# mmetcalf14/qml-cutensornet

Measured on AMD Instinct MI355X. Metric: Gram kernel entries/sec @ 60 qubits x 6 layers, higher is better.
Workload: dtype f64 (complex128)

## Files before the change

qml-cutensornet_amd/csrc/qk_fused.h:

```cpp
#pragma once
#include "qk_device.h"
#include "qk_plan.h"

#define QKF_PRIO_LO() __builtin_amdgcn_s_setprio(0)
#define QKF_PRIO_HI() __builtin_amdgcn_s_setprio(2)
typedef double v2d __attribute__((ext_vector_type(2)));
typedef __attribute__((address_space(3))) v2d lds_v2d;
static constexpr int QKF_XSTEP = 4 * TILE;
static constexpr int QKF_XBLOCK = TILE * TILE;


#ifndef QKF_LDS3M
#define QKF_LDS3M 0
#endif
#ifndef QKF_P2_PROBE
#define QKF_P2_PROBE 0
#endif
#ifndef QKF_ABL
#define QKF_ABL 0
#endif
#define QKF_STEP_BARRIER()                            \
  do {                                                \
    if (QKF_ABL & 4) asm volatile("s_waitcnt lgkmcnt(0)" ::: "memory"); \
    else qk_lds_barrier();                            \
// ... 79 lines not shown
    bo += bs, xq.advance();
#pragma unroll
    for (int i = 0; i < 4; ++i) {
      if (i == 0) {
        const v4d z = {0, 0, 0, 0};
        p1 = __builtin_amdgcn_mfma_f64_16x16x4f64(fx[0].x, fr[0].x, z, 0, 0, 0);
        p2 = __builtin_amdgcn_mfma_f64_16x16x4f64(fx[0].y, fr[0].y, z, 0, 0, 0);
        p3 = __builtin_amdgcn_mfma_f64_16x16x4f64(QKF_SUM(fx[0].x, fx[0].y), QKF_SUM(fr[0].x, fr[0].y), z, 0, 0, 0);
      } else {
        qkf_kstep<false>(p1, p2, p3, fx[i].x, fx[i].y, fr[i].x, fr[i].y);
      }
      if (!(QKF_ABL & 2)) fr[i] = qkf_ldgb(cb[i], bo);
      if (!(QKF_ABL & 8)) fx[i] = xq.kstep(i);
      __builtin_amdgcn_sched_barrier(0);
    }
  }
#pragma unroll 1
  for (int pass = 0; pass < 2; ++pass) {
    const int end = ng - 2 + pass;
#pragma unroll 1
    for (; gq < end; ++gq) {
      bo += bs, xq.advance();
#pragma unroll
      for (int i = 0; i < 4; ++i) {
        qkf_kstep<false>(p1, p2, p3, fx[i].x, fx[i].y, fr[i].x, fr[i].y);
        if (!(QKF_ABL & 2)) fr[i] = qkf_ldgb(cb[i], bo);
        if (!(QKF_ABL & 8)) fx[i] = xq.kstep(i);
        __builtin_amdgcn_sched_barrier(0);
      }
    }
#pragma unroll
    for (int i = 0; i < 4; ++i) cb[i] = qkf_kbase(cur.base, cur.step, i, last);
  }
#pragma unroll
  for (int i = 0; i < 4; ++i) {
    if (i < last) qkf_kstep<false>(p1, p2, p3, fx[i].x, fx[i].y, fr[i].x, fr[i].y);
    if (!(QKF_ABL & 2)) fr[i] = qkf_ldg(qkf_kbase(nxt.base, nxt.step, i, nxt.lim), nxt.off);
    __builtin_amdgcn_sched_barrier(0);
  }
  QKF_PRIO_HI();
  t.re = p1 - p2;
  t.im = p3 - p1 - p2;
}

typedef __attribute__((address_space(3))) int lds_int;
struct QkfTurn {
  lds_int* at;
  int idx;
  lds_int* broken;
  unsigned long long* gerr;
};
__device__ __forceinline__ void qkf_turn_add(__attribute__((address_space(3))) double* const d, const long rs, const v4d& re, const v4d& im, const QkfTurn& t, const int tn) {
  lds_int* const turn = t.at + tn;
  if (t.idx > 0) {
    int spins = 0;
#ifdef QKF_FIRST_STORE
    while (__builtin_amdgcn_readfirstlane(__hip_atomic_load(turn, __ATOMIC_RELAXED, __HIP_MEMORY_SCOPE_WORKGROUP)) == 0) {
#else
    while (__builtin_amdgcn_readfirstlane(__hip_atomic_load(turn, __ATOMIC_RELAXED, __HIP_MEMORY_SCOPE_WORKGROUP)) != t.idx) {
#endif
      __builtin_amdgcn_s_sleep(1);
      if (++spins > (1 << 20) || __builtin_amdgcn_readfirstlane(__hip_atomic_load(t.broken, __ATOMIC_RELAXED, __HIP_MEMORY_SCOPE_WORKGROUP)) != 0) {
        __hip_atomic_store(t.broken, 1, __ATOMIC_RELAXED, __HIP_MEMORY_SCOPE_WORKGROUP);
        if (t.gerr) *t.gerr = 1ull;
        break;
      }
    }
#pragma unroll
    for (int r = 0; r < 4; ++r) {
      __hip_atomic_fetch_add(d + r * rs, re[r], __ATOMIC_RELAXED, __HIP_MEMORY_SCOPE_WORKGROUP);
      __hip_atomic_fetch_add(d + r * rs + 1, im[r], __ATOMIC_RELAXED, __HIP_MEMORY_SCOPE_WORKGROUP);
    }
  } else {
#pragma unroll
    for (int r = 0; r < 4; ++r) *(lds_v2d*)(d + r * rs) = (v2d){re[r], im[r]};
  }
#ifdef QKF_FIRST_STORE
  if (t.idx > 0) return;
#endif
  asm volatile("s_waitcnt lgkmcnt(0)" ::: "memory");
  __hip_atomic_store(turn, t.idx + 1, __ATOMIC_RELAXED, __HIP_MEMORY_SCOPE_WORKGROUP);
}

template <bool FULL, bool DET = false>
__device__ __forceinline__ void qkf_p2_item(const QkfTile& t, v2d (&fr)[4], const bool primed, QkfStream cur, const int ps, const int nn, const int kmax, lds_v2d* xo, const int q,
                                            const int j, const QkfStream nxt, const QkfTurn turn = QkfTurn{nullptr, 0, nullptr, nullptr}) {
  if (!primed) qkf_load4(fr, cur);
  __attribute__((address_space(3))) double* d = (__attribute__((address_space(3))) double*)(xo + q * TILE + j);
  if constexpr (!DET) {
    const v4d z = {0, 0, 0, 0};
    const v4d s = t.re + t.im;
#pragma unroll 1
    for (int tn = 0; tn < nn; ++tn) {
      v4d p1 = z, re, im;
      double sp[4], sm[4];
      const bool fin = tn + 1 == nn;
      const v2d* const rb = fin ? nxt.base : cur.base;
      const int rs = fin ? nxt.step : cur.step, rl = fin ? nxt.lim : FULL ? 4 : kmax;
      cur.off = fin ? nxt.off : cur.off + TILE;
      QKF_PRIO_LO();
#pragma unroll
      for (int i = 0; i < 4; ++i) {
        if (FULL || i == 0 || i < kmax) {
          p1 = __builtin_amdgcn_mfma_f64_16x16x4f64(s[i], fr[i].x, i == 0 ? z : p1, 0, 0, 0);
          sp[i] = QKF_DIF(-fr[i].x, fr[i].y), sm[i] = QKF_DIF(fr[i].y, fr[i].x);
        }
        if (!(QKF_ABL & 2)) fr[i] = qkf_ldg_a(qkf_kbase(rb, rs, i, rl), cur.off);
        __builtin_amdgcn_sched_barrier(0);
      }
#pragma unroll
      for (int i = 0; i < 4; ++i) {
        if (FULL || i == 0 || i < kmax) {
          re = __builtin_amdgcn_mfma_f64_16x16x4f64(t.im[i], sm[i], i == 0 ? p1 : re, 0, 0, 0);
          im = __builtin_amdgcn_mfma_f64_16x16x4f64(t.re[i], sp[i], i == 0 ? p1 : im, 0, 0, 0);
        }
        __builtin_amdgcn_sched_barrier(0);
      }
      QKF_PRIO_HI();
#pragma unroll
      for (int r = 0; r < 4; ++r) {
        __hip_atomic_fetch_add(d + r * 2 * QKF_XSTEP, re[r], __ATOMIC_RELAXED, __HIP_MEMORY_SCOPE_WORKGROUP);
        __hip_atomic_fetch_add(d + r * 2 * QKF_XSTEP + 1, im[r], __ATOMIC_RELAXED, __HIP_MEMORY_SCOPE_WORKGROUP);
      }
      d += 2 * ps;
    }
    return;
  }
#pragma unroll 1
  for (int tn = 0; tn < nn; ++tn) {
    v4d p1 = {0, 0, 0, 0}, p2 = {0, 0, 0, 0}, p3 = {0, 0, 0, 0};
    const bool fin = tn + 1 == nn;
    const v2d* const rb = fin ? nxt.base : cur.base;
    const int rs = fin ? nxt.step : cur.step, rl = fin ? nxt.lim : FULL ? 4 : kmax;
    cur.off = fin ? nxt.off : cur.off + TILE;
    QKF_PRIO_LO();
#pragma unroll
    for (int i = 0; i < 4; ++i) {
      if (FULL || i < kmax) qkf_kstep<true>(p1, p2, p3, t.re[i], t.im[i], fr[i].x, fr[i].y);
      if (!(QKF_ABL & 2)) fr[i] = qkf_ldg_a(qkf_kbase(rb, rs, i, rl), cur.off);
      __builtin_amdgcn_sched_barrier(0);
    }
    QKF_PRIO_HI();
    const v4d re = p1 + p2, im = p3 - p1 + p2;
    qkf_turn_add(d, (long)2 * QKF_XSTEP, re, im, turn, tn);
    d += 2 * ps;
  }
}

template <bool HAS1>
__device__ __forceinline__ void qkf_p2_switch(const QkfTile& t0, const QkfTile& t1, v2d (&fr)[4], const bool primed, QkfStream cur, const int lim, const int nn, const int kmax,
                                              __attribute__((address_space(3))) double* d, const int d1off, const QkfStream nxt) {
  if (!primed) qkf_load4(fr, cur);
  const v4d dm0 = t0.im - t0.re, ng0 = -t0.re - t0.im, dm1 = HAS1 ? t1.im - t1.re : dm0, ng1 = HAS1 ? -t1.re - t1.im : ng0;
#pragma unroll 1
  for (int tn = 0; tn < nn; ++tn) {
    v4d p1 = {0, 0, 0, 0}, p2 = {0, 0, 0, 0}, p3 = {0, 0, 0, 0}, r1 = {0, 0, 0, 0}, r2 = {0, 0, 0, 0}, r3 = {0, 0, 0, 0};
    const bool fin = tn + 1 == nn;
    const v2d* const rb = fin ? nxt.base : cur.base;
    const int rs = fin ? nxt.step : cur.step, rl = fin ? nxt.lim : lim;
    cur.off = fin ? nxt.off : cur.off + TILE;
    QKF_PRIO_LO();
#pragma unroll
    for (int i = 0; i < 4; ++i) {
      if (i < kmax) {
        const double sa = QKF_SUM(fr[i].x, fr[i].y);
        p1 = __builtin_amdgcn_mfma_f64_16x16x4f64(sa, t0.re[i], p1, 0, 0, 0);
        p2 = __builtin_amdgcn_mfma_f64_16x16x4f64(fr[i].y, dm0[i], p2, 0, 0, 0);
        p3 = __builtin_amdgcn_mfma_f64_16x16x4f64(fr[i].x, ng0[i], p3, 0, 0, 0);
        if (HAS1) {
          r1 = __builtin_amdgcn_mfma_f64_16x16x4f64(sa, t1.re[i], r1, 0, 0, 0);
          r2 = __builtin_amdgcn_mfma_f64_16x16x4f64(fr[i].y, dm1[i], r2, 0, 0, 0);
          r3 = __builtin_amdgcn_mfma_f64_16x16x4f64(fr[i].x, ng1[i], r3, 0, 0, 0);
        }
      }
      fr[i] = qkf_ldg_a(qkf_kbase(rb, rs, i, rl), cur.off);
      __builtin_amdgcn_sched_barrier(0);
    }
    QKF_PRIO_HI();
    {
      const v4d re = p1 + p2, im = p1 + p3;
#pragma unroll
      for (int r = 0; r < 4; ++r) {
        __hip_atomic_fetch_add(d + r * 2 * QKF_XSTEP, re[r], __ATOMIC_RELAXED, __HIP_MEMORY_SCOPE_WORKGROUP);
        __hip_atomic_fetch_add(d + r * 2 * QKF_XSTEP + 1, im[r], __ATOMIC_RELAXED, __HIP_MEMORY_SCOPE_WORKGROUP);
      }
    }
    if (HAS1) {
      const v4d re = r1 + r2, im = r1 + r3;
#pragma unroll
      for (int r = 0; r < 4; ++r) {
        __hip_atomic_fetch_add(d + d1off + r * 2 * QKF_XSTEP, re[r], __ATOMIC_RELAXED, __HIP_MEMORY_SCOPE_WORKGROUP);
        __hip_atomic_fetch_add(d + d1off + r * 2 * QKF_XSTEP + 1, im[r], __ATOMIC_RELAXED, __HIP_MEMORY_SCOPE_WORKGROUP);
      }
    }
    d += 2 * QKF_XBLOCK;
  }
}

template <int S>
__device__ __forceinline__ void qkf_rotate(QkfTile (&T)[S], const int L) {
  if constexpr (S >= 2) {
    if (L == 2) {
      const QkfTile t = T[S - 2];
      T[S - 2] = T[S - 1], T[S - 1] = t;
    }
  }
  if constexpr (S >= 3) {
    if (L == 3) {
      const QkfTile t = T[S - 3];
      T[S - 3] = T[S - 2], T[S - 2] = T[S - 1], T[S - 1] = t;
    }
  }
  if constexpr (S >= 4) {
    if (L >= 4) {
      const QkfTile t0 = T[0];
#pragma unroll
      for (int e = 0; e + 1 < S; ++e) T[e] = T[e + 1];
      T[S - 1] = t0;
    }
  }
}

#ifdef QKF_EDGE_PAIRS_V
#define QKF_EDGE_PAIRS(WPS) (QKF_EDGE_PAIRS_V != 0)
#else
#define QKF_EDGE_PAIRS(WPS) false
#endif
#ifdef QKF_EDGE_SETS_V
#define QKF_EDGE_SETS(WPS) (QKF_EDGE_SETS_V)
#else
#define QKF_EDGE_SETS(WPS) ((WPS) <= 3 ? 2 : 1)
#endif
__device__ __forceinline__ v2d qkf_lde(const v2d* __restrict__ base, const unsigned boff, const int col = 0) {
  return reinterpret_cast<const v2d*>(reinterpret_cast<const char*>(base) + (size_t)boff)[col];
}
template <bool HAS1, bool MORE>
__device__ __forceinline__ void qkf_edge_group(v4d (&acc)[6], v2d (&fy)[4], v2d (&fz)[4], v2d (&fx)[4], const v2d* const* const by, const v2d* const* const bx, const unsigned boy,
                                               const unsigned box) {
#pragma unroll
  for (int i = 0; i < 4; ++i) {
    const double sb = QKF_DIF(fx[i].x, fx[i].y);
    acc[0] = __builtin_amdgcn_mfma_f64_16x16x4f64(fy[i].x, fx[i].x, acc[0], 0, 0, 0);
    acc[1] = __builtin_amdgcn_mfma_f64_16x16x4f64(fy[i].y, fx[i].y, acc[1], 0, 0, 0);
    acc[2] = __builtin_amdgcn_mfma_f64_16x16x4f64(QKF_SUM(fy[i].x, fy[i].y), sb, acc[2], 0, 0, 0);
    if (HAS1) {
      acc[3] = __builtin_amdgcn_mfma_f64_16x16x4f64(fz[i].x, fx[i].x, acc[3], 0, 0, 0);
      acc[4] = __builtin_amdgcn_mfma_f64_16x16x4f64(fz[i].y, fx[i].y, acc[4], 0, 0, 0);
      acc[5] = __builtin_amdgcn_mfma_f64_16x16x4f64(QKF_SUM(fz[i].x, fz[i].y), sb, acc[5], 0, 0, 0);
    }
    if (MORE) {
      fy[i] = qkf_lde(by[i], boy);
      if (HAS1) fz[i] = qkf_lde(by[i], boy, TILE);
      fx[i] = qkf_lde(bx[i], box);
    }
    __builtin_amdgcn_sched_barrier(0);
  }
}
template <bool HAS1, int SETS>
__device__ __forceinline__ void qkf_edge_unit(QkfTile& t0, QkfTile& t1, const v2d* __restrict__ Ay, const unsigned oy, const int ldy, const v2d* __restrict__ Ax, const unsigned ox, const int ldx,
                                              const int ng) {
  static_assert(SETS == 1 || SETS == 2, "one or two groups of k-steps in flight");
  v4d acc[6];
#pragma unroll
  for (int e = 0; e < 6; ++e) acc[e] = (v4d){0, 0, 0, 0};
  v2d fy[SETS][4], fz[SETS][4], fx[SETS][4];
  const v2d *by[4 * SETS], *bx[4 * SETS];
#pragma unroll
  for (int i = 0; i < 4 * SETS; ++i) by[i] = Ay + 4 * i * ldy, bx[i] = Ax + 4 * i * ldx;
  unsigned boy = oy * 16u, box = ox * 16u;
  const unsigned sy = (unsigned)(SETS * TILE * ldy) * 16u, sx = (unsigned)(SETS * TILE * ldx) * 16u;
  const bool two = SETS == 2 && ng > 1;
#pragma unroll
  for (int s = 0; s < SETS; ++s) {
    if (s == 0 || two) {
#pragma unroll
      for (int i = 0; i < 4; ++i) {
        fy[s][i] = qkf_lde(by[4 * s + i], boy);
        if (HAS1) fz[s][i] = qkf_lde(by[4 * s + i], boy, TILE);
        fx[s][i] = qkf_lde(bx[4 * s + i], box);
// ... 252 lines not shown
    }
    QKF_STAMP(0);
    QkfTile T[S];
    v2d fr[4];
    bool primed = false;
    QkfSite sn = site(ek);
    for (int k = ek; k < k_hi;) {
      const QkfSite sc = sn;
      k = sc.next;
      if (k < k_hi) sn = site(k);
      const int a = sc.a, a2 = sc.a2, b = sc.b, mt = sc.mt, nt = sc.nt, W = sc.W;
      const bool small = sc.small;
      v2d* const Gc = G0 + (long long)cur * g.x_plane;
      v2d* const Gn = G0 + (long long)(cur ^ 1) * g.x_plane;
      if (small && xg) {
        for (int e = tid; e < a * b; e += NT) XL[e] = Gc[e];
        __syncthreads();
        xg = false, xb = 0;
      } else if (!small && !xg) {
        for (int e = tid; e < a * b; e += NT) Gc[e] = XL[xb + e];
        __syncthreads();
        xg = true;
      }
      const int n_out = sc.b2 * a2;
      const bool pingpong = small && a * b + n_out <= XCAP;
      const int ob = !small ? 0 : pingpong ? (xb == 0 ? XCAP - n_out : 0) : 0;
      if (pingpong && !DET)
        for (int e = tid; e < n_out; e += NT) XL[ob + e] = (v2d){0.0, 0.0};
      QKF_STAMP(1);
      for (int s0 = 0; s0 < nt; s0 += W) {
        const int w = min(W, nt - s0), items = sc.pd * mt * w;
        lds_int* const tcur = turn0 + tsel * g.turn_ints;
        if constexpr (DET) {
          for (int e = tid; e < g.turn_ints; e += NT) turn0[(tsel ^ 1) * g.turn_ints + e] = 0;
        } else if (!small) {
          for (int e = tid; e < w * TILE * a2; e += NT) XL[e] = (v2d){0.0, 0.0};
          QKF_STEP_BARRIER();
        }
        QKF_STAMP(6);
        for (int r0 = 0; r0 < items; r0 += NW * S) {
          const int L = min(S, (items - r0 + NW - 1) / NW);
          const bool multi = L > 1;
          const int it0 = r0 + wave;
          auto phase1 = [&](auto xbase) __attribute__((always_inline)) {
#pragma unroll 1
            for (int s = 0; s < L; ++s) {
              if (multi) qkf_rotate<S>(T, L);
              const int it = it0 + NW * s;
              if (it < items) {
                const int ta = item_of(sc, w, it).ta;
                const bool more = s + 1 < L && it + NW < items;
                const QkfStream nxt = more ? b_stream(sc, s0, w, it + NW) : a_stream(sc, w, it0);
                qkf_p1_tile(T[S - 1], fr, primed, b_stream(sc, s0, w, it), xbase, (unsigned)(ta * (b * TILE) + q * TILE + j), sc.nks, nxt);
                primed = true;
              }
            }
          };
          if (xg) phase1((const v2d*)Gc);
          else phase1((const lds_v2d*)(XL + xb));
          QKF_STAMP(2);
          if (small && r0 == 0 && !(DET && pingpong)) {
            QKF_STEP_BARRIER();
            if (!pingpong && !DET) {
              for (int e = tid; e < n_out; e += NT) XL[e] = (v2d){0.0, 0.0};
              QKF_STEP_BARRIER();
            }
          }
          QKF_STAMP(3);
          const bool last_round = s0 + W >= nt && r0 + NW * S >= items;
#pragma unroll 1
          for (int s = 0; s < S; ++s) {
            const int it = it0 + NW * s;
            if (it >= items) break;
            if (multi) qkf_rotate<S>(T, L);
            const QkUnit un = item_of(sc, w, it);
            const int ta = un.ta, tbl = un.tc;
            const int kmax = min(4, (sc.at - ta * TILE + 3) >> 2);
            const bool more = s + 1 < S && it + NW < items;
            const int wn = min(sn.W, sn.nt);
            const bool chain = !more && last_round && k < k_hi && wave < sn.pd * sn.mt * wn;
            const QkfStream nxt = more ? a_stream(sc, w, it + NW) : chain ? b_stream(sn, 0, wn, wave) : a_stream(sc, w, it);
            const int tix = sc.pd * ta + un.p;
            const QkfTurn turn{tcur + tbl * sc.nn, tix, tbroken, g.err};
            if (!DET && sc.sw)
              qkf_p2_switch<false>(T[S - 1], T[S - 1], fr, primed, a_stream(sc, w, it), kmax, sc.nn, kmax, (__attribute__((address_space(3))) double*)(XL + ob + tbl * (a2 * TILE) + q * TILE + j), 0, nxt);
            else if (kmax == 4) qkf_p2_item<true, DET>(T[S - 1], fr, primed, a_stream(sc, w, it), w * QKF_XBLOCK, sc.nn, 4, XL + ob + tbl * QKF_XBLOCK, q, j, nxt, turn);
            else qkf_p2_item<false, DET>(T[S - 1], fr, primed, a_stream(sc, w, it), w * QKF_XBLOCK, sc.nn, kmax, XL + ob + tbl * QKF_XBLOCK, q, j, nxt, turn);
            primed = more || chain;
          }
          QKF_STAMP(4);
        }
        QKF_STEP_BARRIER();
        tsel ^= 1;
        QKF_STAMP(5);
        if (!small && nt > W) {
          for (int tn = 0; tn < sc.nn; ++tn)
            for (int e = tid; e < w * QKF_XBLOCK; e += NT) Gn[(long long)tn * (sc.b2 * TILE) + s0 * QKF_XBLOCK + e] = XL[tn * w * QKF_XBLOCK + e];
          __syncthreads();
          QKF_STAMP(1);
        }
      }
      if (!small) {
        if (nt > W) cur ^= 1;
        else xg = false, xb = 0;
      } else {
        xb = ob;
      }
    }
    const int fl_end = DET ? 0 : rfl(rec[3 * (k_hi - 1) + 1].w);
    const bool sw_end = (fl_end & QK_REC_SWITCH) != 0, o_end = ((fl_end & QK_REC_ORIENT) != 0) != sw_end;
    if (edges) {
      const v4i r0 = rec[3 * (k_hi - 1)];
      const int a_l = rfl(r0.y), b_l = rfl(r0.w), a_e = sw_end ? b_l : a_l, b_e = sw_end ? a_l : b_l;
      qkf_edge_suffix<NW, QKF_EDGE_PAIRS(WPS), QKF_EDGE_SETS(WPS)>(g, o_end ? yj : xi, o_end ? xi : yj, a_e, b_e, (const lds_v2d*)(XL + xb), (const v2d*)(G0 + (long long)cur * g.x_plane), xg, zacc, wave,
                                                                   q, j, o_end);
      __syncthreads();
    }
    if (tid == 0) {
      v2d zz = {0.0, 0.0};
      if (edges)
        for (int w_ = 0; w_ < NW; ++w_) zz.x += zacc[2 * w_], zz.y += zacc[2 * w_ + 1];
      else zz = xg ? G0[(long long)cur * g.x_plane] : (v2d)XL[xb];
      if (o_end) zz.y = -zz.y;
      g.values[p] = zz.x * zz.x + zz.y * zz.y;
      if (g.z) {
        g.z[2 * p] = zz.x;
        g.z[2 * p + 1] = zz.y;
      }
    }
    __syncthreads();
  }
  if (tid == 0) qk_tail_exit(g);
  QKF_PROF_FLUSH();
}

template <bool HAS1, typename XPtr>
__device__ __forceinline__ void qkf_p1_dual(QkfTile& t0, QkfTile& t1, v2d (&fr)[4], v2d (&fs)[4], const bool primed, QkfStream cur, XPtr xp, unsigned xoff, const int nks,
                                            const QkfStream nxt) {
  v4d p1 = {0, 0, 0, 0}, p2 = {0, 0, 0, 0}, p3 = {0, 0, 0, 0}, r1 = {0, 0, 0, 0}, r2 = {0, 0, 0, 0}, r3 = {0, 0, 0, 0};
  v2d fx[4];
  if (!primed) qkf_load4(fr, cur);
  if (HAS1) {
#pragma unroll
    for (int i = 0; i < 4; ++i) fs[i] = qkf_ldg(cur.base + i * cur.step, cur.off + TILE);
  }
#pragma unroll
  for (int i = 0; i < 4; ++i) fx[i] = qkf_ldx(xp + i * QKF_XSTEP, xoff);
  const int ng = (nks + 3) >> 2, last = nks - 4 * (ng - 1);
  QKF_PRIO_LO();
  int gq = 0;
  if (ng >= 2) {
    gq = 1;
    cur.off += 4 * cur.step, xoff += 4 * QKF_XSTEP;
#pragma unroll
    for (int i = 0; i < 4; ++i) {
      if (i == 0) {
        const v4d z = {0, 0, 0, 0};
        const double sa = QKF_SUM(fx[0].x, fx[0].y);
        p1 = __builtin_amdgcn_mfma_f64_16x16x4f64(fx[0].x, fr[0].x, z, 0, 0, 0);
        p2 = __builtin_amdgcn_mfma_f64_16x16x4f64(fx[0].y, fr[0].y, z, 0, 0, 0);
        p3 = __builtin_amdgcn_mfma_f64_16x16x4f64(sa, QKF_SUM(fr[0].x, fr[0].y), z, 0, 0, 0);
        if (HAS1) {
          r1 = __builtin_amdgcn_mfma_f64_16x16x4f64(fx[0].x, fs[0].x, z, 0, 0, 0);
          r2 = __builtin_amdgcn_mfma_f64_16x16x4f64(fx[0].y, fs[0].y, z, 0, 0, 0);
          r3 = __builtin_amdgcn_mfma_f64_16x16x4f64(sa, QKF_SUM(fs[0].x, fs[0].y), z, 0, 0, 0);
        }
      } else {
        qkf_kstep<false>(p1, p2, p3, fx[i].x, fx[i].y, fr[i].x, fr[i].y);
        if (HAS1) qkf_kstep<false>(r1, r2, r3, fx[i].x, fx[i].y, fs[i].x, fs[i].y);
      }
      if (!(QKF_ABL & 2)) fr[i] = qkf_ldg_b(cur.base + i * cur.step, cur.off);
      if (HAS1 && !(QKF_ABL & 2)) fs[i] = qkf_ldg_b(cur.base + i * cur.step, cur.off + TILE);
      if (!(QKF_ABL & 8)) fx[i] = qkf_ldx(xp + i * QKF_XSTEP, xoff);
      __builtin_amdgcn_sched_barrier(0);
    }
  }
#pragma unroll 1
  for (; gq + 1 < ng; ++gq) {
    cur.off += 4 * cur.step, xoff += 4 * QKF_XSTEP;
#pragma unroll
    for (int i = 0; i < 4; ++i) {
      qkf_kstep<false>(p1, p2, p3, fx[i].x, fx[i].y, fr[i].x, fr[i].y);
      if (HAS1) qkf_kstep<false>(r1, r2, r3, fx[i].x, fx[i].y, fs[i].x, fs[i].y);
      if (!(QKF_ABL & 2)) fr[i] = qkf_ldg_b(cur.base + i * cur.step, cur.off);
      if (HAS1 && !(QKF_ABL & 2)) fs[i] = qkf_ldg_b(cur.base + i * cur.step, cur.off + TILE);
      if (!(QKF_ABL & 8)) fx[i] = qkf_ldx(xp + i * QKF_XSTEP, xoff);
      __builtin_amdgcn_sched_barrier(0);
    }
  }
#pragma unroll
  for (int i = 0; i < 4; ++i) {
    if (i < last) {
      qkf_kstep<false>(p1, p2, p3, fx[i].x, fx[i].y, fr[i].x, fr[i].y);
      if (HAS1) qkf_kstep<false>(r1, r2, r3, fx[i].x, fx[i].y, fs[i].x, fs[i].y);
    }
    if (!(QKF_ABL & 2)) fr[i] = qkf_ldg(nxt.base + i * nxt.step, nxt.off);
    __builtin_amdgcn_sched_barrier(0);
  }
  QKF_PRIO_HI();
  t0.re = p1 - p2, t0.im = p3 - p1 - p2;
  if (HAS1) t1.re = r1 - r2, t1.im = r3 - r1 - r2;
}

typedef __attribute__((address_space(3))) double lds_double;
template <bool FULL, bool HAS1>
__device__ __forceinline__ void qkf_p2_block(const QkfTile& t0, const QkfTile& t1, const v4d& s0, const v4d& s1, v2d (&fr)[4], const int kmax, const v2d* const b0, const v2d* const b1,
                                             const v2d* const b2, const v2d* const b3, const unsigned off, lds_double* const d, lds_double* const d1, const long rs) {
  const v4d z = {0, 0, 0, 0};
  v4d p1 = z, r1 = z, re, im, re1, im1;
  double sp[4], sm[4];
  QKF_PRIO_LO();
#pragma unroll
  for (int i = 0; i < 4; ++i) {
    if (FULL || i == 0 || i < kmax) {
      p1 = __builtin_amdgcn_mfma_f64_16x16x4f64(s0[i], fr[i].x, i == 0 ? z : p1, 0, 0, 0);
      if (HAS1) r1 = __builtin_amdgcn_mfma_f64_16x16x4f64(s1[i], fr[i].x, i == 0 ? z : r1, 0, 0, 0);
      sp[i] = QKF_DIF(-fr[i].x, fr[i].y), sm[i] = QKF_DIF(fr[i].y, fr[i].x);
    }
    if (!(QKF_ABL & 2)) fr[i] = qkf_ldg_a(i == 0 ? b0 : i == 1 ? b1 : i == 2 ? b2 : b3, off);
    __builtin_amdgcn_sched_barrier(0);
  }
#pragma unroll
  for (int i = 0; i < 4; ++i) {
    if (FULL || i == 0 || i < kmax) {
      re = __builtin_amdgcn_mfma_f64_16x16x4f64(t0.im[i], sm[i], i == 0 ? p1 : re, 0, 0, 0);
      im = __builtin_amdgcn_mfma_f64_16x16x4f64(t0.re[i], sp[i], i == 0 ? p1 : im, 0, 0, 0);
      if (HAS1) {
        re1 = __builtin_amdgcn_mfma_f64_16x16x4f64(t1.im[i], sm[i], i == 0 ? r1 : re1, 0, 0, 0);
        im1 = __builtin_amdgcn_mfma_f64_16x16x4f64(t1.re[i], sp[i], i == 0 ? r1 : im1, 0, 0, 0);
      }
    }
    __builtin_amdgcn_sched_barrier(0);
  }
  QKF_PRIO_HI();
#pragma unroll
  for (int r = 0; r < 4; ++r) {
    __hip_atomic_fetch_add(d + r * rs, re[r], __ATOMIC_RELAXED, __HIP_MEMORY_SCOPE_WORKGROUP);
    __hip_atomic_fetch_add(d + r * rs + 1, im[r], __ATOMIC_RELAXED, __HIP_MEMORY_SCOPE_WORKGROUP);
  }
  if (HAS1) {
#pragma unroll
    for (int r = 0; r < 4; ++r) {
      __hip_atomic_fetch_add(d1 + r * rs, re1[r], __ATOMIC_RELAXED, __HIP_MEMORY_SCOPE_WORKGROUP);
      __hip_atomic_fetch_add(d1 + r * rs + 1, im1[r], __ATOMIC_RELAXED, __HIP_MEMORY_SCOPE_WORKGROUP);
    }
  }
}
template <bool FULL, bool HAS1, bool DET>
__device__ __forceinline__ void qkf_p2_dual_turn(const QkfTile& t0, const QkfTile& t1, v2d (&fr)[4], v2d (&fs)[4], QkfStream cur, const int ps, const int nn, const int kmax, lds_v2d* xo, const int q,
                                            const int j, const QkfStream nxt, const bool nxt_p1, const unsigned n1, const QkfTurn turn = QkfTurn{nullptr, 0, nullptr, nullptr}) {
  __attribute__((address_space(3))) double* d = (__attribute__((address_space(3))) double*)(xo + q * TILE + j);
#pragma unroll 1
  for (int tn = 0; tn < nn; ++tn) {
    v4d p1 = {0, 0, 0, 0}, p2 = {0, 0, 0, 0}, p3 = {0, 0, 0, 0}, r1 = {0, 0, 0, 0}, r2 = {0, 0, 0, 0}, r3 = {0, 0, 0, 0};
    const bool fin = tn + 1 == nn;
    const v2d* const rb = fin ? nxt.base : cur.base;
    const int rs = fin ? nxt.step : cur.step;
    cur.off = fin ? nxt.off : cur.off + TILE;
    QKF_PRIO_LO();
#pragma unroll
    for (int i = 0; i < 4; ++i) {
      if (FULL || i < kmax) {
        qkf_kstep<true>(p1, p2, p3, t0.re[i], t0.im[i], fr[i].x, fr[i].y);
        if (HAS1) qkf_kstep<true>(r1, r2, r3, t1.re[i], t1.im[i], fr[i].x, fr[i].y);
      }
      fr[i] = qkf_ldg_a(rb + i * rs, cur.off);
      __builtin_amdgcn_sched_barrier(0);
    }
    QKF_PRIO_HI();
    {
      const v4d re = p1 + p2, im = p3 - p1 + p2;
      if constexpr (DET) qkf_turn_add(d, (long)2 * QKF_XSTEP, re, im, turn, tn);
      else {
#pragma unroll
        for (int r = 0; r < 4; ++r) {
          __hip_atomic_fetch_add(d + r * 2 * QKF_XSTEP, re[r], __ATOMIC_RELAXED, __HIP_MEMORY_SCOPE_WORKGROUP);
          __hip_atomic_fetch_add(d + r * 2 * QKF_XSTEP + 1, im[r], __ATOMIC_RELAXED, __HIP_MEMORY_SCOPE_WORKGROUP);
        }
      }
    }
    if (HAS1) {
      const v4d re = r1 + r2, im = r3 - r1 + r2;
      __attribute__((address_space(3))) double* const d1 = d + 2 * QKF_XBLOCK;
      if constexpr (DET) qkf_turn_add(d1, (long)2 * QKF_XSTEP, re, im, QkfTurn{turn.at + nn, turn.idx, turn.broken, turn.gerr}, tn);
      else {
#pragma unroll
        for (int r = 0; r < 4; ++r) {
          __hip_atomic_fetch_add(d1 + r * 2 * QKF_XSTEP, re[r], __ATOMIC_RELAXED, __HIP_MEMORY_SCOPE_WORKGROUP);
          __hip_atomic_fetch_add(d1 + r * 2 * QKF_XSTEP + 1, im[r], __ATOMIC_RELAXED, __HIP_MEMORY_SCOPE_WORKGROUP);
        }
      }
    }
    d += 2 * ps;
  }
}

template <bool FULL, bool HAS1, bool DET = false>
__device__ __forceinline__ void qkf_p2_dual(const QkfTile& t0, const QkfTile& t1, v2d (&fr)[4], v2d (&fs)[4], QkfStream cur, const int ps, const int nn, const int kmax, lds_v2d* xo, const int q,
                                            const int j, const QkfStream nxt, const bool nxt_p1, const unsigned n1, const QkfTurn turn = QkfTurn{nullptr, 0, nullptr, nullptr}) {
  if constexpr (DET) {
    qkf_p2_dual_turn<FULL, HAS1, DET>(t0, t1, fr, fs, cur, ps, nn, kmax, xo, q, j, nxt, nxt_p1, n1, turn);
    return;
  }
  lds_double* d = (lds_double*)(xo + q * TILE + j);
  lds_double* d1 = d + 2 * QKF_XBLOCK;
  constexpr long rs = 2 * QKF_XSTEP;
  const v4d s0 = t0.re + t0.im, s1 = HAS1 ? t1.re + t1.im : s0;
  const v2d *const c0 = cur.base, *const c1 = cur.base + cur.step, *const c2 = cur.base + 2 * cur.step, *const c3 = cur.base + 3 * cur.step;
  unsigned off = cur.off;
#pragma unroll 1
  for (int tn = 0; tn + 1 < nn; ++tn) {
    off += TILE;
    qkf_p2_block<FULL, HAS1>(t0, t1, s0, s1, fr, kmax, c0, c1, c2, c3, off, d, d1, rs);
    d += 2 * ps, d1 += 2 * ps;
  }
  qkf_p2_block<FULL, HAS1>(t0, t1, s0, s1, fr, kmax, nxt.base, nxt.base + nxt.step, nxt.base + 2 * nxt.step, nxt.base + 3 * nxt.step, nxt.off, d, d1, rs);
}

template <int NW, int XCAP, int WPS, bool DET = false>
__global__ __launch_bounds__(64 * NW, WPS) void qk_sweep_fused_dual_kernel(const SweepArgs g) {
  constexpr int NT = 64 * NW;
  extern __shared__ __attribute__((aligned(16))) double lds_raw[];
  lds_v2d* const XL = (lds_v2d*)lds_raw;
  long long* const slot = reinterpret_cast<long long*>(lds_raw + 2 * XCAP);
  const v2d* const xdata = reinterpret_cast<const v2d*>(g.xdata);
  const v2d* const ydata = reinterpret_cast<const v2d*>(g.ydata);
  v2d* const G0 = reinterpret_cast<v2d*>(g.scratch) + (long long)blockIdx.x * 2 * g.x_plane;
  const int tid = threadIdx.x, lane = tid & 63;
  const int wave = __builtin_amdgcn_readfirstlane(tid >> 6);
  const int j = lane & 15, q = lane >> 4;
  const int ns = g.n_sites;
  __attribute__((address_space(3))) double* const zacc = (__attribute__((address_space(3))) double*)(slot + 2);
  lds_v4i* const rec = (lds_v4i*)(slot + 2 + 32);
  long long* const m_off = reinterpret_cast<long long*>(slot + 2 + 32) + 6 * (long long)ns;
  lds_int* const tbroken = (lds_int*)(m_off + 2 * (long long)ns);
  lds_int* const turn0 = tbroken + 2;
  auto rfl = [&](const int v) __attribute__((always_inline)) { return __builtin_amdgcn_readfirstlane(v); };
  auto ldl = [&](const long long* p_) __attribute__((always_inline)) {
    const long long v = *p_;
    const unsigned lo = __builtin_amdgcn_readfirstlane((unsigned)v);
    const unsigned hi = __builtin_amdgcn_readfirstlane((unsigned)((unsigned long long)v >> 32));
    return (long long)(((unsigned long long)hi << 32) | lo);
  };
  auto site = [&](const int k) __attribute__((always_inline)) {
    const v4i r0 = rec[3 * k], r1 = rec[3 * k + 1], r2 = rec[3 * k + 2];
    QkfSite s;
    s.a = rfl(r0.x), s.a2 = rfl(r0.y), s.b = rfl(r0.z), s.b2 = rfl(r0.w);
    s.at = rfl(r1.x), s.nks = rfl(r1.y), s.W = rfl(r1.z), s.small = (rfl(r1.w) & QK_REC_SMALL) != 0, s.sw = (rfl(r1.w) & QK_REC_SWITCH) != 0;
    s.inv = rfl(r2.x);
    s.ps = rfl(r2.y), s.pd = 1 << s.ps, s.next = rfl(r2.z);
    s.mt = s.a / TILE, s.nt = s.b2 / TILE, s.nn = s.a2 / TILE;
    s.Ak = xdata + ldl(m_off + 2 * k);
    s.Bk = ydata + ldl(m_off + 2 * k + 1);
    return s;
  };
  auto pair_of = [&](const QkfSite& s, const int v) __attribute__((always_inline)) { return qk_unit_decode_ordered(v, s.ps, s.mt, s.inv); };
  auto b_stream = [&](const QkfSite& s, const int s0, const int v, const int half) __attribute__((always_inline)) {
    const QkUnit un = pair_of(s, v);
    return QkfStream{s.Bk + un.p * s.b2, (unsigned)((q * s.pd) * s.b2 + (s0 + 2 * un.tc + half) * TILE + j), 4 * s.pd * s.b2};
  };
  struct Unit {
    bool mine, has1;
    int v, half;
  };
  auto unit_of = [&](const QkfSite& s, const int w, const int units, const int r0) __attribute__((always_inline)) {
    Unit un;
    const int left = units - r0;
    const bool halves = 2 * left <= NW;
    un.half = (halves && wave >= left) ? 1 : 0;
    un.v = r0 + wave - (un.half ? left : 0);
    const int tp = pair_of(s, un.v).tc;
    const bool second = 2 * tp + 1 < w;
    un.mine = un.v < units && (un.half == 0 || second);
    un.has1 = !halves && second;
    return un;
  };
  auto a_stream = [&](const QkfSite& s, const int v) __attribute__((always_inline)) {
    const QkUnit un = pair_of(s, v);
    return QkfStream{s.Ak + un.p * s.a2, (unsigned)(((un.ta * TILE + q) * s.pd) * s.a2 + j), 4 * s.pd * s.a2};
  };
  QKF_PROF_DECL();
  const int xcc = qk_xcc_id();
  int gang_round = 0;
  if (tid == 0) qk_tail_start(g);
  if (tid == QKF_PULLER(NT)) qkf_pull_next(g, xcc, gang_round, slot);
  __syncthreads();
  long long p = slot[0];
  int psel = 0;
// ... 27 lines not shown
    QkfTile T0, T1;
    v2d fr[4], fs[4];
    bool primed = false;
    QkfSite sn = site(ek);
    for (int k = ek; k < k_hi;) {
      const QkfSite sc = sn;
      k = sc.next;
      if (k < k_hi) sn = site(k);
      const int a = sc.a, a2 = sc.a2, b = sc.b, mt = sc.mt, nt = sc.nt, W = sc.W;
      const bool small = sc.small;
      v2d* const Gc = G0 + (long long)cur * g.x_plane;
      v2d* const Gn = G0 + (long long)(cur ^ 1) * g.x_plane;
      if (small && xg) {
        for (int e = tid; e < a * b; e += NT) XL[e] = Gc[e];
        __syncthreads();
        xg = false, xb = 0;
      } else if (!small && !xg) {
        for (int e = tid; e < a * b; e += NT) Gc[e] = XL[xb + e];
        __syncthreads();
        xg = true;
      }
      const int n_out = sc.b2 * a2;
      const bool pingpong = small && a * b + n_out <= XCAP;
      const int ob = !small ? 0 : pingpong ? (xb == 0 ? XCAP - n_out : 0) : 0;
      if (pingpong && !DET)
        for (int e = tid; e < n_out; e += NT) XL[ob + e] = (v2d){0.0, 0.0};
      QKF_STAMP(1);
      for (int s0 = 0; s0 < nt; s0 += W) {
        const int w = min(W, nt - s0), units = sc.pd * mt * ((w + 1) >> 1);
        lds_int* const tcur = turn0 + tsel * g.turn_ints;
        if constexpr (DET) {
          for (int e = tid; e < g.turn_ints; e += NT) turn0[(tsel ^ 1) * g.turn_ints + e] = 0;
        } else if (!small) {
          for (int e = tid; e < w * TILE * a2; e += NT) XL[e] = (v2d){0.0, 0.0};
          QKF_STEP_BARRIER();
        }
        for (int r0 = 0; r0 < units; r0 += NW) {
          const Unit un = unit_of(sc, w, units, r0);
          const int v = un.v;
          const bool mine = un.mine, has1 = un.has1;
          const QkUnit pr = pair_of(sc, v);
          const int tp = pr.tc, ta = pr.ta;
          if (mine) {
            const QkfStream bs = b_stream(sc, s0, v, un.half), as = a_stream(sc, v);
            const unsigned xoff = (unsigned)(ta * (b * TILE) + q * TILE + j);
            if (xg) {
              if (has1) qkf_p1_dual<true>(T0, T1, fr, fs, primed, bs, (const v2d*)Gc, xoff, sc.nks, as);
              else qkf_p1_dual<false>(T0, T1, fr, fs, primed, bs, (const v2d*)Gc, xoff, sc.nks, as);
            } else {
              if (has1) qkf_p1_dual<true>(T0, T1, fr, fs, primed, bs, (const lds_v2d*)(XL + xb), xoff, sc.nks, as);
              else qkf_p1_dual<false>(T0, T1, fr, fs, primed, bs, (const lds_v2d*)(XL + xb), xoff, sc.nks, as);
            }
          }
          QKF_STAMP(2);
          if (small && r0 == 0 && !(DET && pingpong)) {
            QKF_STEP_BARRIER();
            if (!pingpong && !DET) {
              for (int e = tid; e < n_out; e += NT) XL[e] = (v2d){0.0, 0.0};
              QKF_STEP_BARRIER();
            }
          }
          QKF_STAMP(3);
          if (mine) {
            const int kmax = min(4, (sc.at - ta * TILE + 3) >> 2);
            QkfStream nxt = a_stream(sc, v);
            bool np1 = false;
            if (r0 + NW < units) {
              const Unit nu = unit_of(sc, w, units, r0 + NW);
              if (nu.mine) nxt = b_stream(sc, s0, nu.v, nu.half), np1 = true;
            } else if (s0 + W < nt) {
              const int w2 = min(W, nt - s0 - W);
              const Unit nu = unit_of(sc, w2, sc.pd * mt * ((w2 + 1) >> 1), 0);
              if (nu.mine) nxt = b_stream(sc, s0 + W, nu.v, nu.half), np1 = true;
            } else if (k < k_hi) {
              const int w2 = min(sn.W, sn.nt);
              const Unit nu = unit_of(sn, w2, sn.pd * sn.mt * ((w2 + 1) >> 1), 0);
              if (nu.mine) nxt = b_stream(sn, 0, nu.v, nu.half), np1 = true;
            }
            const unsigned nd1 = 0;
            lds_v2d* const xo = XL + ob + (2 * tp + un.half) * QKF_XBLOCK;
            const QkfTurn tp_turn{tcur + (2 * tp + un.half) * sc.nn, sc.pd * ta + pr.p, tbroken, g.err};
            if (!DET && sc.sw) {
              lds_double* const dsw = (lds_double*)(XL + ob + (2 * tp + un.half) * (a2 * TILE) + q * TILE + j);
              if (has1) qkf_p2_switch<true>(T0, T1, fr, true, a_stream(sc, v), 4, sc.nn, kmax, dsw, 2 * a2 * TILE, nxt);
              else qkf_p2_switch<false>(T0, T1, fr, true, a_stream(sc, v), 4, sc.nn, kmax, dsw, 0, nxt);
            } else if (has1) {
              if (kmax == 4) qkf_p2_dual<true, true, DET>(T0, T1, fr, fs, a_stream(sc, v), w * QKF_XBLOCK, sc.nn, 4, xo, q, j, nxt, np1, nd1, tp_turn);
              else qkf_p2_dual<false, true, DET>(T0, T1, fr, fs, a_stream(sc, v), w * QKF_XBLOCK, sc.nn, kmax, xo, q, j, nxt, np1, nd1, tp_turn);
            } else {
              if (kmax == 4) qkf_p2_dual<true, false, DET>(T0, T1, fr, fs, a_stream(sc, v), w * QKF_XBLOCK, sc.nn, 4, xo, q, j, nxt, np1, nd1, tp_turn);
              else qkf_p2_dual<false, false, DET>(T0, T1, fr, fs, a_stream(sc, v), w * QKF_XBLOCK, sc.nn, kmax, xo, q, j, nxt, np1, nd1, tp_turn);
            }
            primed = np1;
          }
          QKF_STAMP(4);
        }
        QKF_STEP_BARRIER();
        tsel ^= 1;
        QKF_STAMP(5);
        if (!small && nt > W) {
          for (int tn = 0; tn < sc.nn; ++tn)
            for (int e = tid; e < w * QKF_XBLOCK; e += NT) Gn[(long long)tn * (sc.b2 * TILE) + s0 * QKF_XBLOCK + e] = XL[tn * w * QKF_XBLOCK + e];
          __syncthreads();
        }
      }
      if (!small) {
        if (nt > W) cur ^= 1;
        else xg = false, xb = 0;
      } else {
        xb = ob;
      }
    }
    if (tid == QKF_PULLER(NT)) qkf_pull_next(g, xcc, gang_round, slot + (psel ^ 1));
    const int fl_end = DET ? 0 : rfl(rec[3 * (k_hi - 1) + 1].w);
    const bool sw_end = (fl_end & QK_REC_SWITCH) != 0, o_end = ((fl_end & QK_REC_ORIENT) != 0) != sw_end;
    if (edges) {
      const v4i r0 = rec[3 * (k_hi - 1)];
      const int a_l = rfl(r0.y), b_l = rfl(r0.w), a_e = sw_end ? b_l : a_l, b_e = sw_end ? a_l : b_l;
      qkf_edge_suffix<NW, QKF_EDGE_PAIRS(WPS), QKF_EDGE_SETS(WPS)>(g, o_end ? yj : xi, o_end ? xi : yj, a_e, b_e, (const lds_v2d*)(XL + xb), (const v2d*)(G0 + (long long)cur * g.x_plane), xg, zacc, wave,
                                                                   q, j, o_end);
    }
    __syncthreads();
    const long long pn = slot[psel ^ 1];
    if (tid == 0) {
      v2d zz = {0.0, 0.0};
      if (edges)
        for (int w_ = 0; w_ < NW; ++w_) zz.x += zacc[2 * w_], zz.y += zacc[2 * w_ + 1];
      else zz = xg ? G0[(long long)cur * g.x_plane] : (v2d)XL[xb];
      if (o_end) zz.y = -zz.y;
      g.values[p] = zz.x * zz.x + zz.y * zz.y;
      if (g.z) {
        g.z[2 * p] = zz.x;
        g.z[2 * p + 1] = zz.y;
      }
    }
    table_of(pn);
    if (!edges) __syncthreads();
    p = pn, psel ^= 1;
    QKF_STAMP(6);
  }
  if (tid == 0) qk_tail_exit(g);
  QKF_PROF_FLUSH();
}

template <typename T>
__global__ void qk_interleave_kernel(const T* __restrict__ src, T* __restrict__ dst, const int32_t* __restrict__ dims, const int64_t* __restrict__ offs,
                                     const int n_sites, const long long n_tensors) {
  typedef T v2 __attribute__((ext_vector_type(2)));
  for (long long t = blockIdx.x; t < n_tensors; t += gridDim.x) {
    const long long s = t / n_sites;
    const int k = (int)(t - s * n_sites);
    const long long plane = (long long)dims[s * (n_sites + 1) + k] * 2 * dims[s * (n_sites + 1) + k + 1];
    const T* re = src + offs[t];
    const T* im = re + plane;
    v2* d = reinterpret_cast<v2*>(dst + offs[t]);
    for (long long e = threadIdx.x; e < plane; e += blockDim.x) d[e] = (v2){re[e], im[e]};
  }
}

template <int N>
__device__ __forceinline__ void qkw_wait_vmcnt() {
  static_assert(N >= 0 && N < 64, "vmcnt is a 6-bit field");
  asm volatile("s_waitcnt vmcnt(%0)" ::"n"(N) : "memory");
}

template <int NG, typename SRC>
__global__ __launch_bounds__(64, 2) void qk_sweep_wave2_kernel(const SweepArgs g) {
  constexpr bool F32 = sizeof(SRC) == 4;
// ... 198 lines not shown
```

Baseline: 762,800.

## Unify phase-2 complex products into single-sum chained MFMA form

Adds a shared phase-2 block routine that computes the complex tile product with a 3-MFMA-chain formulation. The shared sum term seeds the accumulators of the real and imaginary chains, so fewer accumulators and final adds are needed. The routine replaces the normal, dual and switch phase-2 paths by default through compile-time form macros. Next-tile loads are interleaved with the MFMAs and pinned with empty asm. This aims to cut register pressure and vector ALU work, but the serial dependency chain could lengthen MFMA latency exposure.

```diff
diff --git a/qml-cutensornet_amd/csrc/qk_fused.h b/qml-cutensornet_amd/csrc/qk_fused.h
--- a/qml-cutensornet_amd/csrc/qk_fused.h
+++ b/qml-cutensornet_amd/csrc/qk_fused.h
@@ -185,11 +185,114 @@
   __hip_atomic_store(turn, t.idx + 1, __ATOMIC_RELAXED, __HIP_MEMORY_SCOPE_WORKGROUP);
 }
 
-template <bool FULL, bool DET = false>
+#ifndef QKF_P2_FORM_DUAL
+#define QKF_P2_FORM_DUAL 1
+#endif
+#ifndef QKF_P2_FORM_ONE
+#define QKF_P2_FORM_ONE 1
+#endif
+#ifndef QKF_P2_FORM_TWO
+#define QKF_P2_FORM_TWO 1
+#endif
+typedef __attribute__((address_space(3))) double lds_double;
+struct QkfTSet {
+  v4d k, a, b;
+};
+template <bool SWITCH>
+__device__ __forceinline__ QkfTSet qkf_tset(const QkfTile& t) {
+  return SWITCH ? QkfTSet{t.re, t.im - t.re, -t.re - t.im} : QkfTSet{t.im, t.re - t.im, -t.re - t.im};
+}
+template <bool SWITCH>
+__device__ __forceinline__ v4d qkf_p2_mma(const double t, const double f, const v4d& c) {
+  return SWITCH ? __builtin_amdgcn_mfma_f64_16x16x4f64(f, t, c, 0, 0, 0) : __builtin_amdgcn_mfma_f64_16x16x4f64(t, f, c, 0, 0, 0);
+}
+#define QKF_PIN2(a, b) asm volatile("" : "+v"(a), "+v"(b) : : "memory")
+template <bool FULL, bool HAS1, bool SWITCH>
+__device__ __forceinline__ void qkf_p2_onesum(const QkfTSet& u0, const QkfTSet& u1, v2d (&fa)[4], const int kmax, const v2d* const b0, const v2d* const b1, const v2d* const b2,
+                                              const v2d* const b3, const unsigned off, lds_double* const d, lds_double* const d1) {
+  constexpr long rs = 2 * QKF_XSTEP;
+  const v4d z = {0, 0, 0, 0};
+  v4d p1 = z, r1 = z, re, im, re1, im1;
+  QKF_PRIO_LO();
+  double s = QKF_SUM(fa[0].x, fa[0].y);
+#pragma unroll
+  for (int i = 0; i < 4; ++i) {
+    if (FULL || i == 0 || i < kmax) {
+      p1 = qkf_p2_mma<SWITCH>(u0.k[i], s, i == 0 ? z : p1);
+      if (HAS1) r1 = qkf_p2_mma<SWITCH>(u1.k[i], s, i == 0 ? z : r1);
+    }
+    if (i < 3) s = QKF_SUM(fa[i + 1].x, fa[i + 1].y);
+    __builtin_amdgcn_sched_barrier(0);
+  }
+#pragma unroll
+  for (int i = 0; i < 4; ++i) {
+    if (FULL || i == 0 || i < kmax) {
+      const double fre = SWITCH ? fa[i].y : fa[i].x, fim = SWITCH ? fa[i].x : fa[i].y;
+      re = qkf_p2_mma<SWITCH>(u0.a[i], fre, i == 0 ? p1 : re);
+      im = qkf_p2_mma<SWITCH>(u0.b[i], fim, i == 0 ? p1 : im);
+    }
+    if (!HAS1 && !(QKF_ABL & 2)) {
+      QKF_PIN2(re, im);
+      fa[i] = qkf_ldg_a(i == 0 ? b0 : i == 1 ? b1 : i == 2 ? b2 : b3, off);
+    }
+    __builtin_amdgcn_sched_barrier(0);
+  }
+  if (HAS1) {
+    QKF_PIN2(re, im);
+#pragma unroll
+    for (int i = 0; i < 4; ++i) {
+      if (FULL || i == 0 || i < kmax) {
+        const double fre = SWITCH ? fa[i].y : fa[i].x, fim = SWITCH ? fa[i].x : fa[i].y;
+        re1 = qkf_p2_mma<SWITCH>(u1.a[i], fre, i == 0 ? r1 : re1);
+        im1 = qkf_p2_mma<SWITCH>(u1.b[i], fim, i == 0 ? r1 : im1);
+      }
+      if (!(QKF_ABL & 2)) {
+        QKF_PIN2(re1, im1);
+        fa[i] = qkf_ldg_a(i == 0 ? b0 : i == 1 ? b1 : i == 2 ? b2 : b3, off);
+      }
+      __builtin_amdgcn_sched_barrier(0);
+    }
+  }
+  QKF_PRIO_HI();
+#pragma unroll
+  for (int r = 0; r < 4; ++r) {
+    __hip_atomic_fetch_add(d + r * rs, re[r], __ATOMIC_RELAXED, __HIP_MEMORY_SCOPE_WORKGROUP);
+    __hip_atomic_fetch_add(d + r * rs + 1, im[r], __ATOMIC_RELAXED, __HIP_MEMORY_SCOPE_WORKGROUP);
+  }
+  if (HAS1) {
+#pragma unroll
+    for (int r = 0; r < 4; ++r) {
+      __hip_atomic_fetch_add(d1 + r * rs, re1[r], __ATOMIC_RELAXED, __HIP_MEMORY_SCOPE_WORKGROUP);
+      __hip_atomic_fetch_add(d1 + r * rs + 1, im1[r], __ATOMIC_RELAXED, __HIP_MEMORY_SCOPE_WORKGROUP);
+    }
+  }
+}
+template <bool FULL, bool HAS1, bool SWITCH>
+__device__ __forceinline__ void qkf_p2_blocks(const QkfTile& t0, const QkfTile& t1, v2d (&fr)[4], const QkfStream cur, const int lim, const QkfStream nxt, const int nn, const int kmax,
+                                              lds_double* d, const int d1off, const int dstep) {
+  const QkfTSet u0 = qkf_tset<SWITCH>(t0), u1 = HAS1 ? qkf_tset<SWITCH>(t1) : u0;
+  const v2d *const c0 = qkf_kbase(cur.base, cur.step, 0, lim), *const c1 = qkf_kbase(cur.base, cur.step, 1, lim), *const c2 = qkf_kbase(cur.base, cur.step, 2, lim),
+            *const c3 = qkf_kbase(cur.base, cur.step, 3, lim);
+  unsigned off = cur.off;
+#pragma unroll 1
+  for (int tn = 0; tn + 1 < nn; ++tn) {
+    off += TILE;
+    qkf_p2_onesum<FULL, HAS1, SWITCH>(u0, u1, fr, kmax, c0, c1, c2, c3, off, d, d + d1off);
+    d += dstep;
+  }
+  qkf_p2_onesum<FULL, HAS1, SWITCH>(u0, u1, fr, kmax, qkf_kbase(nxt.base, nxt.step, 0, nxt.lim), qkf_kbase(nxt.base, nxt.step, 1, nxt.lim), qkf_kbase(nxt.base, nxt.step, 2, nxt.lim),
+                                    qkf_kbase(nxt.base, nxt.step, 3, nxt.lim), nxt.off, d, d + d1off);
+}
+
+template <bool FULL, bool DET = false, int FORM = 0>
 __device__ __forceinline__ void qkf_p2_item(const QkfTile& t, v2d (&fr)[4], const bool primed, QkfStream cur, const int ps, const int nn, const int kmax, lds_v2d* xo, const int q,
                                             const int j, const QkfStream nxt, const QkfTurn turn = QkfTurn{nullptr, 0, nullptr, nullptr}) {
   if (!primed) qkf_load4(fr, cur);
   __attribute__((address_space(3))) double* d = (__attribute__((address_space(3))) double*)(xo + q * TILE + j);
+  if constexpr (!DET && FORM != 0) {
+    qkf_p2_blocks<FULL, false, false>(t, t, fr, cur, FULL ? 4 : kmax, nxt, nn, kmax, d, 0, 2 * ps);
+    return;
+  }
   if constexpr (!DET) {
     const v4d z = {0, 0, 0, 0};
     const v4d s = t.re + t.im;
@@ -251,9 +354,8 @@
 }
 
 template <bool HAS1>
-__device__ __forceinline__ void qkf_p2_switch(const QkfTile& t0, const QkfTile& t1, v2d (&fr)[4], const bool primed, QkfStream cur, const int lim, const int nn, const int kmax,
-                                              __attribute__((address_space(3))) double* d, const int d1off, const QkfStream nxt) {
-  if (!primed) qkf_load4(fr, cur);
+__device__ __forceinline__ void qkf_p2_switch_simple(const QkfTile& t0, const QkfTile& t1, v2d (&fr)[4], QkfStream cur, const int lim, const int nn, const int kmax,
+                                                     __attribute__((address_space(3))) double* d, const int d1off, const QkfStream nxt) {
   const v4d dm0 = t0.im - t0.re, ng0 = -t0.re - t0.im, dm1 = HAS1 ? t1.im - t1.re : dm0, ng1 = HAS1 ? -t1.re - t1.im : ng0;
 #pragma unroll 1
   for (int tn = 0; tn < nn; ++tn) {
@@ -298,6 +400,13 @@
     }
     d += 2 * QKF_XBLOCK;
   }
+}
+template <bool FULL, bool HAS1, int FORM>
+__device__ __forceinline__ void qkf_p2_switch(const QkfTile& t0, const QkfTile& t1, v2d (&fr)[4], const bool primed, const QkfStream cur, const int lim, const int nn, const int kmax,
+                                              lds_double* const d, const int d1off, const QkfStream nxt) {
+  if (!primed) qkf_load4(fr, cur);
+  if constexpr (FORM == 0) qkf_p2_switch_simple<HAS1>(t0, t1, fr, cur, lim, nn, kmax, d, d1off, nxt);
+  else qkf_p2_blocks<FULL, HAS1, true>(t0, t1, fr, cur, lim, nxt, nn, kmax, d, d1off, 2 * QKF_XBLOCK);
 }
 
 template <int S>
@@ -716,10 +825,13 @@
             const QkfStream nxt = more ? a_stream(sc, w, it + NW) : chain ? b_stream(sn, 0, wn, wave) : a_stream(sc, w, it);
             const int tix = sc.pd * ta + un.p;
             const QkfTurn turn{tcur + tbl * sc.nn, tix, tbroken, g.err};
-            if (!DET && sc.sw)
-              qkf_p2_switch<false>(T[S - 1], T[S - 1], fr, primed, a_stream(sc, w, it), kmax, sc.nn, kmax, (__attribute__((address_space(3))) double*)(XL + ob + tbl * (a2 * TILE) + q * TILE + j), 0, nxt);
-            else if (kmax == 4) qkf_p2_item<true, DET>(T[S - 1], fr, primed, a_stream(sc, w, it), w * QKF_XBLOCK, sc.nn, 4, XL + ob + tbl * QKF_XBLOCK, q, j, nxt, turn);
-            else qkf_p2_item<false, DET>(T[S - 1], fr, primed, a_stream(sc, w, it), w * QKF_XBLOCK, sc.nn, kmax, XL + ob + tbl * QKF_XBLOCK, q, j, nxt, turn);
+            constexpr int FORM = DET ? 0 : WPS >= 4 ? QKF_P2_FORM_TWO : QKF_P2_FORM_ONE;
+            if (!DET && sc.sw) {
+              lds_double* const dsw = (lds_double*)(XL + ob + tbl * (a2 * TILE) + q * TILE + j);
+              if (FORM != 0 && kmax == 4) qkf_p2_switch<true, false, FORM>(T[S - 1], T[S - 1], fr, primed, a_stream(sc, w, it), 4, sc.nn, 4, dsw, 0, nxt);
+              else qkf_p2_switch<false, false, FORM>(T[S - 1], T[S - 1], fr, primed, a_stream(sc, w, it), kmax, sc.nn, kmax, dsw, 0, nxt);
+            } else if (kmax == 4) qkf_p2_item<true, DET, FORM>(T[S - 1], fr, primed, a_stream(sc, w, it), w * QKF_XBLOCK, sc.nn, 4, XL + ob + tbl * QKF_XBLOCK, q, j, nxt, turn);
+            else qkf_p2_item<false, DET, FORM>(T[S - 1], fr, primed, a_stream(sc, w, it), w * QKF_XBLOCK, sc.nn, kmax, XL + ob + tbl * QKF_XBLOCK, q, j, nxt, turn);
             primed = more || chain;
           }
           QKF_STAMP(4);
@@ -836,7 +948,6 @@
   if (HAS1) t1.re = r1 - r2, t1.im = r3 - r1 - r2;
 }
 
-typedef __attribute__((address_space(3))) double lds_double;
 template <bool FULL, bool HAS1>
 __device__ __forceinline__ void qkf_p2_block(const QkfTile& t0, const QkfTile& t1, const v4d& s0, const v4d& s1, v2d (&fr)[4], const int kmax, const v2d* const b0, const v2d* const b1,
                                              const v2d* const b2, const v2d* const b3, const unsigned off, lds_double* const d, lds_double* const d1, const long rs) {
@@ -938,6 +1049,10 @@
   }
   lds_double* d = (lds_double*)(xo + q * TILE + j);
   lds_double* d1 = d + 2 * QKF_XBLOCK;
+  if constexpr (QKF_P2_FORM_DUAL != 0) {
+    qkf_p2_blocks<FULL, HAS1, false>(t0, t1, fr, cur, 4, nxt, nn, kmax, d, 2 * QKF_XBLOCK, 2 * ps);
+    return;
+  }
   constexpr long rs = 2 * QKF_XSTEP;
   const v4d s0 = t0.re + t0.im, s1 = HAS1 ? t1.re + t1.im : s0;
   const v2d *const c0 = cur.base, *const c1 = cur.base + cur.step, *const c2 = cur.base + 2 * cur.step, *const c3 = cur.base + 3 * cur.step;
@@ -1131,8 +1246,14 @@
             const QkfTurn tp_turn{tcur + (2 * tp + un.half) * sc.nn, sc.pd * ta + pr.p, tbroken, g.err};
             if (!DET && sc.sw) {
               lds_double* const dsw = (lds_double*)(XL + ob + (2 * tp + un.half) * (a2 * TILE) + q * TILE + j);
-              if (has1) qkf_p2_switch<true>(T0, T1, fr, true, a_stream(sc, v), 4, sc.nn, kmax, dsw, 2 * a2 * TILE, nxt);
-              else qkf_p2_switch<false>(T0, T1, fr, true, a_stream(sc, v), 4, sc.nn, kmax, dsw, 0, nxt);
+              constexpr int FORM = QKF_P2_FORM_DUAL;
+              if (FORM != 0 && kmax == 4) {
+                if (has1) qkf_p2_switch<true, true, FORM>(T0, T1, fr, true, a_stream(sc, v), 4, sc.nn, 4, dsw, 2 * a2 * TILE, nxt);
+                else qkf_p2_switch<true, false, FORM>(T0, T1, fr, true, a_stream(sc, v), 4, sc.nn, 4, dsw, 0, nxt);
+              } else {
+                if (has1) qkf_p2_switch<false, true, FORM>(T0, T1, fr, true, a_stream(sc, v), 4, sc.nn, kmax, dsw, 2 * a2 * TILE, nxt);
+                else qkf_p2_switch<false, false, FORM>(T0, T1, fr, true, a_stream(sc, v), 4, sc.nn, kmax, dsw, 0, nxt);
+              }
             } else if (has1) {
               if (kmax == 4) qkf_p2_dual<true, true, DET>(T0, T1, fr, fs, a_stream(sc, v), w * QKF_XBLOCK, sc.nn, 4, xo, q, j, nxt, np1, nd1, tp_turn);
               else qkf_p2_dual<false, true, DET>(T0, T1, fr, fs, a_stream(sc, v), w * QKF_XBLOCK, sc.nn, kmax, xo, q, j, nxt, np1, nd1, tp_turn);
```

New measurement: 774,600, median of 6. 1.6% higher.
